# DIAGNijmegen/bodyct-dram-emph-subtype

Measured on AMD Instinct MI355X. Metric: CT volumes/sec (train step, 1x128x256x256), higher is better.
Workload: dtype f32; 1 GPU; BASELINE configs[1]: resnet18segcls train step (fwd+loss+bwd+Adam), batch 2/GPU, 1x128x256x256, fp32, inputs resident in HBM; global_batch=2, parallelism=dp1, hip_graph=False, streams=2

## Files before the change

bodyct-dram-emph-subtype_amd/csrc/conv_wino.hip:

```cpp
#include <stdio.h>
#include <stdlib.h>
#include <string.h>
#include "common.h"

namespace {

struct WinoGeom {
  int B, D, H, W;
  int d;
  int nz, ny, nx;
  int npts;
  int Tz, Ty, Tx;
  int T;
  int Tpad;
};

__device__ __forceinline__ void tile_origin(const WinoGeom& g, int t, int& b, int& z0, int& y0, int& x0) {
  int r = t;
  const int tx = r % g.Tx; r /= g.Tx;
  const int ty = r % g.Ty; r /= g.Ty;
  const int tz = r % g.Tz; r /= g.Tz;
  const int rx = r % g.d; r /= g.d;
  const int ry = r % g.d; r /= g.d;
  const int rz = r % g.d;
// ... 1432 lines not shown
  const int tid = threadIdx.x;
  const int lane = tid & 63;
  const int wave = __builtin_amdgcn_readfirstlane(tid >> 6);
  int L = xcd_remap(blockIdx.x, nblk);
  const int nt = L % n_tiles; L /= n_tiles;
  const int mt = L % m_tiles; L /= m_tiles;
  const int split = L % nsplit;
  const int xi = L / nsplit;
  const int t0 = split * kper;
  const int t1 = (t0 + kper < Tpad) ? t0 + kper : Tpad;
  int bcol = nt * BN + (lane % BQ) * 4;
  if (bcol > N - 4) bcol = N - 4;
  const float* Ab = Ah + (long)(lane / AQ) * M + mt * BM + (lane % AQ) * 4;
  const float* Bb = Bh + (long)(lane / BQ) * N + bcol;

  auto issue = [&](int it, int stage) __attribute__((always_inline)) {
    float* as = lds + stage * STAGE;
    float* bs = as + 32 * BM;
    const int tt = t0 + it * 32;
    const long row = ((long)(tt >> 8) * npts + xi) * 256 + (tt & 255);
    const float* ag = Ab + row * M;
    const float* bg = Bb + row * N;
#pragma unroll
    for (int j = 0; j < APW; ++j) {
      const int p = APW * wave + j;
      __builtin_amdgcn_global_load_lds((const __attribute__((address_space(1))) void*)(ag + (long)(p * ARPP) * M),
                                       (__attribute__((address_space(3))) void*)(as + p * 256), 16, 0, 0);
    }
#pragma unroll
    for (int jj = 0; jj < BPW; ++jj) {
      const int p = BPW * wave + jj;
      __builtin_amdgcn_global_load_lds((const __attribute__((address_space(1))) void*)(bg + (long)(p * BRPP) * N),
                                       (__attribute__((address_space(3))) void*)(bs + p * 256), 16, 0, 0);
    }
  };

  f32x16 acc[MI][NJ];
#pragma unroll
  for (int mi = 0; mi < MI; ++mi)
#pragma unroll
    for (int nj = 0; nj < NJ; ++nj)
#pragma unroll
      for (int e = 0; e < 16; ++e) acc[mi][nj][e] = 0.f;

  const int li = lane & 31, lh = lane >> 5;
  const int wm = wave % WMW, wn = wave / WMW;
  const int niter = (t1 - t0) / 32;

  if (niter > 0) issue(0, 0);
  for (int it = 0; it < niter; ++it) {
    __syncthreads();
    if (it + 1 < niter) issue(it + 1, (it + 1) & 1);
    const float* as = lds + (it & 1) * STAGE + wm * 32 * MI + li;
    const float* bs = lds + (it & 1) * STAGE + 32 * BM + wn * 32 * NJ + li;
#pragma unroll 4
    for (int kk = 0; kk < 16; ++kk) {
      const int kr = 2 * kk + lh;
      float af[MI], bf[NJ];
#pragma unroll
      for (int mi = 0; mi < MI; ++mi) af[mi] = as[kr * BM + mi * 32];
#pragma unroll
      for (int nj = 0; nj < NJ; ++nj) bf[nj] = bs[kr * BN + nj * 32];
#pragma unroll
      for (int nj = 0; nj < NJ; ++nj)
#pragma unroll
        for (int mi = 0; mi < MI; ++mi)
          acc[mi][nj] = __builtin_amdgcn_mfma_f32_32x32x2f32(af[mi], bf[nj], acc[mi][nj], 0, 0, 0);
    }
  }

  float* sb = slab + (((long)split * npts + xi) * M + mt * BM) * N + nt * BN;
#pragma unroll
  for (int mi = 0; mi < MI; ++mi)
#pragma unroll
    for (int e = 0; e < 16; ++e) {
      const int row = wm * 32 * MI + mi * 32 + (e & 3) + 8 * (e >> 2) + 4 * lh;
      float* o = sb + (long)row * N + wn * 32 * NJ + li;
#pragma unroll
      for (int nj = 0; nj < NJ; ++nj)
        if (nt * BN + wn * 32 * NJ + nj * 32 + li < N) o[nj * 32] = acc[mi][nj][e];
    }
}

__global__ __launch_bounds__(512, 2) void wino_gemm_tn64_kernel(const float* __restrict__ Ah, const float* __restrict__ Bh,
                                                                float* __restrict__ slab, const int Tpad, const int nsplit,
                                                                const int kper, const int nblk, const int npts) {
  constexpr int M = 64, N = 64, KS = 64;
  constexpr int STAGE = KS * (M + N);
  __shared__ __attribute__((aligned(1024))) float lds[2 * STAGE];
  const int tid = threadIdx.x, lane = tid & 63;
  const int wave = __builtin_amdgcn_readfirstlane(tid >> 6);
  int L = xcd_remap(blockIdx.x, nblk);
  const int split = L % nsplit;
  const int xi = L / nsplit;
  const int t0 = split * kper;
  const int t1 = (t0 + kper < Tpad) ? t0 + kper : Tpad;
  const int prow = lane >> 4, pcol = (lane & 15) * 4;
  auto issue = [&](int it, int stage) __attribute__((always_inline)) {
    float* as = lds + stage * STAGE;
    float* bs = as + KS * M;
    const int tt = t0 + it * KS;
    const long row = ((long)(tt >> 8) * npts + xi) * 256 + (tt & 255);
#pragma unroll
    for (int j = 0; j < 2; ++j) {
      const int p = 2 * wave + j;
      __builtin_amdgcn_global_load_lds((const __attribute__((address_space(1))) void*)(Ah + (row + p * 4 + prow) * M + pcol),
                                       (__attribute__((address_space(3))) void*)(as + p * 256), 16, 0, 0);
      __builtin_amdgcn_global_load_lds((const __attribute__((address_space(1))) void*)(Bh + (row + p * 4 + prow) * N + pcol),
                                       (__attribute__((address_space(3))) void*)(bs + p * 256), 16, 0, 0);
    }
  };
  f32x16 acc;
#pragma unroll
  for (int e = 0; e < 16; ++e) acc[e] = 0.f;
  const int li = lane & 31, lh = lane >> 5;
  const int wm = wave & 1, wn = (wave >> 1) & 1, kh = wave >> 2;
  const int niter = (t1 - t0) / KS;
  if (niter > 0) issue(0, 0);
  for (int it = 0; it < niter; ++it) {
    __syncthreads();
    if (it + 1 < niter) issue(it + 1, (it + 1) & 1);
    const float* as = lds + (it & 1) * STAGE + (kh * 32) * M + wm * 32 + li;
    const float* bs = lds + (it & 1) * STAGE + KS * M + (kh * 32) * N + wn * 32 + li;
#pragma unroll 4
    for (int kk = 0; kk < 16; ++kk) {
      const int kr = 2 * kk + lh;
      acc = __builtin_amdgcn_mfma_f32_32x32x2f32(as[kr * M], bs[kr * N], acc, 0, 0, 0);
    }
  }
  __syncthreads();
  float* ex = lds + (wave & 3) * 1024;
  if (kh == 1) {
#pragma unroll
    for (int e = 0; e < 16; ++e) ex[e * 64 + lane] = acc[e];
  }
  __syncthreads();
  if (kh == 0) {
    float* sb = slab + (((long)split * npts + xi) * M) * N;
#pragma unroll
    for (int e = 0; e < 16; ++e) {
      const int row = wm * 32 + (e & 3) + 8 * (e >> 2) + 4 * lh;
      sb[(long)row * N + wn * 32 + li] = acc[e] + ex[e * 64 + lane];
    }
  }
}

typedef short s16x4 __attribute__((ext_vector_type(4)));
typedef short s16x8 __attribute__((ext_vector_type(8)));

template <int WMW, int MI, int NJ, int NT>
__global__ __launch_bounds__(512) void wino_gemm_tn_bf16_kernel(const float* __restrict__ Ah, const float* __restrict__ Bh,
                                                                float* __restrict__ slab, const int Tpad, const int M,
                                                                const int N, const int m_tiles, const int n_tiles,
                                                                const int nsplit, const int kper, const int nblk,
                                                                const int npts) {
  constexpr int WNW = 8 / WMW;
  constexpr int BM = WMW * 32 * MI, BN = WNW * 32 * NJ;
  static_assert(BM % 64 == 0 && BM <= 256 && BN % 64 == 0 && BN <= 256, "one DMA piece = 256 floats");
  constexpr int STAGE = 32 * (BM + BN);
  constexpr int AQ = BM / 4, ARPP = 64 / AQ, APW = BM / 64;
  constexpr int BQ = BN / 4, BRPP = 64 / BQ, BPW = BN / 64;
  __shared__ __attribute__((aligned(1024))) float lds[2 * STAGE];

  const int tid = threadIdx.x;
  const int lane = tid & 63;
  const int wave = __builtin_amdgcn_readfirstlane(tid >> 6);
// ... 118 lines not shown
      for (int nj = 0; nj < NJ; ++nj)
        if (nt * BN + wn * 32 * NJ + nj * 32 + li < N) o[nj * 32] = acc[mi][nj][e];
    }
}

#define WINO_TILING_DISPATCH(g_, CALL_)                                 \
  do {                                                                  \
    if ((g_).nz == 4 && (g_).ny == 4 && (g_).nx == 4) { CALL_(4, 4, 4); } \
    else if ((g_).nz == 4 && (g_).ny == 4) { CALL_(4, 4, 2); }          \
    else if ((g_).nz == 4) { CALL_(4, 2, 2); }                          \
    else { CALL_(2, 2, 2); }                                            \
  } while (0)
int math_mode() {
  const char* e = tune_env("DRAM_MATH");
  if (!e) return 0;
  if (!strcmp(e, "bf16x3")) return 1;
  if (!strcmp(e, "bf16")) return 2;
  return 0;
}

bool wino_geom_ok(const DramConvDesc* d) {
  if (!d) return false;
  if (d->B < 1 || d->D < 1 || d->H < 1 || d->W < 1) return false;
  if (d->k != 3 || d->stride != 1 || d->dil < 1 || d->pad != d->dil) return false;
  if (d->Do != d->D || d->Ho != d->H || d->Wo != d->W) return false;
  if (d->Cin < 64 || d->Cout < 64 || d->Cin % 64 != 0 || d->Cout % 64 != 0) return false;
  return true;
}

long long tiles_for(const DramConvDesc* d, int nz, int ny, int nx) {
  const int dd = d->dil;
  auto tiles = [&](int n, int per) { return (long long)(((n + dd - 1) / dd + per - 1) / per); };
  return (long long)d->B * dd * dd * dd * tiles(d->D, nz) * tiles(d->H, ny) * tiles(d->W, nx);
}

void pick_tiling(const DramConvDesc* d, const int pass, int& nz, int& ny, int& nx) {
  static const int cand[4][3] = {{4, 4, 4}, {4, 4, 2}, {4, 2, 2}, {2, 2, 2}};
  if (const char* e = tune_env("DRAM_WINO_TILING")) {
    int a = 0, b = 0, c = 0;
    if (sscanf(e, "%d,%d,%d", &a, &b, &c) == 3)
      for (int i = 0; i < 4; ++i)
        if (cand[i][0] == a && cand[i][1] == b && cand[i][2] == c) { nz = a; ny = b; nx = c; return; }
  }
  if (math_mode() == 2) { nz = ny = nx = 2; return; }
  (void)pass;
  long long best = -1;
  int bi = 3;
  for (int i = 0; i < 4; ++i) {
    const long long T = tiles_for(d, cand[i][0], cand[i][1], cand[i][2]);
    const long long Tpad = (T + 255) / 256 * 256;
    if (i < 3 && Tpad < 512) continue;
    const long long cost = (long long)(cand[i][0] + 2) * (cand[i][1] + 2) * (cand[i][2] + 2) * (Tpad + T);
    if (best < 0 || cost < best) { best = cost; bi = i; }
  }
  nz = cand[bi][0]; ny = cand[bi][1]; nx = cand[bi][2];
}

WinoGeom make_geom(const DramConvDesc* d, const int pass = 0) {
  WinoGeom g{};
  g.B = d->B; g.D = d->D; g.H = d->H; g.W = d->W; g.d = d->dil;
  pick_tiling(d, pass, g.nz, g.ny, g.nx);
  g.npts = (g.nz + 2) * (g.ny + 2) * (g.nx + 2);
  auto tiles = [&](int n, int per) { return ((n + g.d - 1) / g.d + per - 1) / per; };
  g.Tz = tiles(g.D, g.nz); g.Ty = tiles(g.H, g.ny); g.Tx = tiles(g.W, g.nx);
  const long long T = (long long)g.B * g.d * g.d * g.d * g.Tz * g.Ty * g.Tx;
  g.T = (int)T;
  g.Tpad = (int)((T + 255) / 256 * 256);
  return g;
}

bool wino_size_ok(const DramConvDesc* d) {
  const long long cmax = d->Cin > d->Cout ? d->Cin : d->Cout;
  for (int pass = 0; pass < 2; ++pass) {
    const WinoGeom g = make_geom(d, pass);
    const long long T = (long long)g.B * g.d * g.d * g.d * g.Tz * g.Ty * g.Tx;
    if (!(T > 0 && (T + 255) * cmax < (1LL << 31))) return false;
  }
  const long long plane_b = (long long)d->H * d->W * cmax * 4;
  if ((5LL * d->dil + 1) * plane_b >= (1LL << 30) || 216LL * 256 * cmax * 4 >= (1LL << 30)) return false;
  return true;
}


struct TnPlan { int bm, bn, m_tiles, n_tiles, nsplit, kper; };
bool plan_tn(const DramConvDesc* d, const WinoGeom& g, TnPlan& p) {
  const int M = d->Cout, N = d->Cin;
  p.bm = M % 256 == 0 ? 256 : (M % 128 == 0 ? 128 : 64);
  const int ncand = p.bm == 256 ? 3 : 2;
  const int cand[3] = {256, 128, 64};
  p.bn = 0;
  int best_pad = 1 << 30;
  for (int i = 0; i < ncand; ++i) {
    const int padded = (N + cand[i] - 1) / cand[i] * cand[i];
    if (padded * 100 <= N * 113) { p.bn = cand[i]; break; }
    if (padded < best_pad) { best_pad = padded; p.bn = cand[i]; }
  }
  p.m_tiles = M / p.bm;
  p.n_tiles = (N + p.bn - 1) / p.bn;
  if (p.bn >= 128 && (p.bn > 128 || p.bm == 256)) {
    const long w1 = (long)g.npts * p.m_tiles * p.n_tiles;
    const int hb = p.bn / 2, hn = (N + hb - 1) / hb;
    const long w2 = (long)g.npts * p.m_tiles * hn;
    if (w1 >= 512 && (double)((w2 + 255) / 256) * 0.5 * 1.03 < (double)((w1 + 255) / 256)) {
      p.bn = hb;
      p.n_tiles = hn;
    }
  }
  const int base = g.npts * p.m_tiles * p.n_tiles;
  const int k32 = g.Tpad / 32;
  int ns = 1;
  while (base * ns < (g.npts == 1 ? 256 : 512) && ns * 2 <= k32 / 4 && ns < (g.npts == 1 ? 256 : 16)) ns *= 2;
  p.nsplit = ns;
  p.kper = ((k32 + ns - 1) / ns) * 32;
  return true;
}

int wino_nt() {
  static const int v = tune_env("DRAM_WINO_NT") ? atoi(tune_env("DRAM_WINO_NT")) : 3;
  return v;
}

int grid_for(long waves) {
  long b = (waves + 3) / 4;
  return (int)(b > 65536 ? 65536 : (b < 1 ? 1 : b));
}

template <int MODE>
int launch_wino_in(const float* src, float* dst, const WinoGeom& g, const int C, const int math, hipStream_t s,
                   const float* pscale = nullptr, const float* pshift = nullptr, const int Cd = 0, const int cofs = 0) {
  const long units = (long)g.Tpad * (C / 64);
  if (Cd && (math || !(g.nz == 4 && g.ny == 4 && g.nx == 4) || C % 64 || cofs % 64 || cofs + C > Cd)) return DRAM_ERR_UNSUPPORTED;
  if (pscale) {
    if (MODE != 0 || math || !pshift || !(g.nz == 4 && g.ny == 4 && g.nx == 4)) return DRAM_ERR_UNSUPPORTED;
    const double in_elems = (double)g.B * g.D * g.H * g.W * C;
    DramProf prof(DRAM_FAM_WINO_IN, 9444, 0.0, 4.0 * (in_elems + (double)g.npts * g.Tpad * C), s);
    if constexpr (MODE == 0) {
      if (wino_nt() & 1) hipLaunchKernelGGL((wino_in444_kernel<0, false, true, true>), dim3(grid_for(2 * units)), dim3(256), 0, s, src, dst, g, C, pscale, pshift, Cd, cofs);
      else hipLaunchKernelGGL((wino_in444_kernel<0, false, false, true>), dim3(grid_for(2 * units)), dim3(256), 0, s, src, dst, g, C, pscale, pshift, Cd, cofs);
    }
    DRAM_LAUNCH_CHECK();
    return DRAM_OK;
  }
  const double in_elems = (double)g.B * g.D * g.H * g.W * C;
  DramProf prof(DRAM_FAM_WINO_IN, MODE * 1000 + g.nz * 100 + g.ny * 10 + g.nx, 0.0,
                4.0 * (in_elems + (double)g.npts * g.Tpad * C), s);
  static const int half = tune_env("DRAM_WINO_HALF") ? atoi(tune_env("DRAM_WINO_HALF")) : 1;
  if ((half || Cd) && g.nz == 4 && g.ny == 4 && g.nx == 4) {
    if (math) hipLaunchKernelGGL((wino_in444_kernel<MODE, true, false>), dim3(grid_for(2 * units)), dim3(256), 0, s, src, dst, g, C, nullptr, nullptr, 0, 0);
    else if (wino_nt() & 1) hipLaunchKernelGGL((wino_in444_kernel<MODE, false, true>), dim3(grid_for(2 * units)), dim3(256), 0, s, src, dst, g, C, nullptr, nullptr, Cd, cofs);
    else hipLaunchKernelGGL((wino_in444_kernel<MODE, false, false>), dim3(grid_for(2 * units)), dim3(256), 0, s, src, dst, g, C, nullptr, nullptr, Cd, cofs);
    DRAM_LAUNCH_CHECK();
    return DRAM_OK;
  }
#define W_IN1(NZ_, NY_, NX_)                                                                                       \
  do {                                                                                                             \
    if (math)                                                                                                      \
      hipLaunchKernelGGL((wino_in_kernel<MODE, NZ_, NY_, NX_, true>), dim3(grid_for(units)), dim3(256), 0, s, src, dst, g, C);  \
    else                                                                                                           \
      hipLaunchKernelGGL((wino_in_kernel<MODE, NZ_, NY_, NX_, false>), dim3(grid_for(units)), dim3(256), 0, s, src, dst, g, C); \
  } while (0)
  WINO_TILING_DISPATCH(g, W_IN1);
#undef W_IN1
  DRAM_LAUNCH_CHECK();
  return DRAM_OK;
}

int run_nn(const float* A, const float* U, float* Y, const WinoGeom& g, int N, int K, hipStream_t s,
           const GemmEpilogue ep = GemmEpilogue{nullptr, nullptr, nullptr, nullptr}, const int math = 0,
           const bool alone = true) {
  const int m_tiles = g.Tpad / 256;
  int nj = 1;
  double best = 1e30;
  for (int c = 4; c >= 1; c >>= 1) {
    if (N % (64 * c) != 0) continue;
    const long wgs = (long)g.npts * m_tiles * (N / (64 * c));
    const double cost = (double)((wgs + 255) / 256) * c * (c == 4 ? 1.0 : (c == 2 ? 1.03 : 1.10));
    if (cost < best) { best = cost; nj = c; }
  }
  if (const char* e = tune_env("DRAM_NN_NJ")) { const int v = atoi(e); if ((v == 1 || v == 2 || v == 4) && N % (64 * v) == 0) nj = v; }
  const int n_tiles = N / (64 * nj);
  const int nblk = g.npts * m_tiles * n_tiles;
  DramProf prof(DRAM_FAM_WINO_GEMM_NN, nj, 2.0 * g.npts * (double)g.Tpad * N * K,
                4.0 * g.npts * ((double)g.Tpad * (K + N) + (double)N * K), s,
                g.npts > 1 ? 2.0 * g.B * g.D * g.H * g.W * (double)N * K * 27.0 : -1.0);
  if (math) {
#define WNB(NJ_, NT_)                                                                                                  \
  hipLaunchKernelGGL((wino_gemm_nn_bf16_kernel<NJ_, NT_>), dim3(nblk), dim3(512), 0, s, A, U, Y, g.Tpad, N, K, m_tiles, \
                     n_tiles, nblk, g.npts)
    if (math == 1) { if (nj == 4) WNB(4, 3); else if (nj == 2) WNB(2, 3); else WNB(1, 3); }
    else { if (nj == 4) WNB(4, 1); else if (nj == 2) WNB(2, 1); else WNB(1, 1); }
#undef WNB
    DRAM_LAUNCH_CHECK();
    return DRAM_OK;
  }
#define WNN(NJ_)                                                                                                   \
  hipLaunchKernelGGL((wino_gemm_nn_kernel<NJ_>), dim3(nblk), dim3(512), 0, s, A, U, Y, g.Tpad, N, K, m_tiles, n_tiles, \
                     nblk, g.npts, ep, epi_lds)
// ... 127 lines not shown
  if (d->Cin < 64 || d->Cout < 64 || d->Cin % 64 != 0 || d->Cout % 64 != 0) return false;
  const long long M = (long long)d->B * d->D * d->H * d->W;
  const long long cmax = d->Cin > d->Cout ? d->Cin : d->Cout;
  return M % 256 == 0 && M * cmax < (1LL << 31);
}
WinoGeom c1_geom(const DramConvDesc* d) {
  WinoGeom g{};
  g.B = d->B; g.D = d->D; g.H = d->H; g.W = d->W; g.d = 1;
  g.nz = g.ny = g.nx = 1;
  g.npts = 1;
  g.T = g.Tpad = d->B * d->D * d->H * d->W;
  return g;
}
__global__ __launch_bounds__(256) void slab_sum_kernel(const float* __restrict__ slab, float* __restrict__ out, const long n,
                                                       const int nsplit) {
  __shared__ float part[4][64];
  const int r = threadIdx.x & 63, kg = threadIdx.x >> 6;
  for (long i0 = blockIdx.x * 64L; i0 < n; i0 += (long)gridDim.x * 64L) {
    const long i = i0 + r;
    const bool live = i < n;
    float p[8];
#pragma unroll
    for (int j = 0; j < 8; ++j) p[j] = 0.f;
    if (live) {
      int k = kg;
      for (; k + 28 < nsplit; k += 32) {
#pragma unroll
        for (int j = 0; j < 8; ++j) p[j] += slab[(long)(k + 4 * j) * n + i];
      }
      for (int j = 0; k < nsplit; k += 4, ++j) p[j] += slab[(long)k * n + i];
    }
    part[kg][r] = ((p[0] + p[1]) + (p[2] + p[3])) + ((p[4] + p[5]) + (p[6] + p[7]));
    __syncthreads();
    if (kg == 0 && live) out[i] = (part[0][r] + part[1][r]) + (part[2][r] + part[3][r]);
    __syncthreads();
  }
}
}

extern "C" int dram_conv1x1_applicable(const DramConvDesc* d) { return c1_ok(d) ? 1 : 0; }

extern "C" int dram_conv1x1_num_stat_rows(const DramConvDesc* d) {
  if (!c1_ok(d)) return DRAM_ERR_UNSUPPORTED;
  return c1_geom(d).Tpad / 256;
}

extern "C" int dram_conv1x1_fwd(const float* x, const float* w2d, const float* bias, float* y, float* stats_partial,
                                const DramConvDesc* d, dram_stream_t stream) {
  if (!x || !w2d || !y) return DRAM_ERR_BAD_ARG;
  if (!c1_ok(d)) return DRAM_ERR_UNSUPPORTED;
  return run_nn(x, w2d, y, c1_geom(d), d->Cout, d->Cin, (hipStream_t)stream,
                GemmEpilogue{bias, nullptr, nullptr, stats_partial});
}

extern "C" int dram_conv1x1_bwd_data(const float* dy, const float* wt, float* dx, const float* add, const float* gate,
                                     const DramConvDesc* d, dram_stream_t stream) {
  if (!dy || !wt || !dx || (gate && !add)) return DRAM_ERR_BAD_ARG;
  if (!c1_ok(d)) return DRAM_ERR_UNSUPPORTED;
  return run_nn(dy, wt, dx, c1_geom(d), d->Cin, d->Cout, (hipStream_t)stream, GemmEpilogue{nullptr, add, gate, nullptr});
}

extern "C" size_t dram_conv1x1_bwd_weight_workspace(const DramConvDesc* d) {
  if (!c1_ok(d)) return 0;
  TnPlan p;
  plan_tn(d, c1_geom(d), p);
  return (size_t)p.nsplit * d->Cout * d->Cin * sizeof(float);
}

extern "C" int dram_conv1x1_bwd_weight(const float* x, const float* dy, float* dw, const DramConvDesc* d, void* workspace,
                                       size_t workspace_bytes, dram_stream_t stream) {
  if (!x || !dy || !dw) return DRAM_ERR_BAD_ARG;
  if (!c1_ok(d)) return DRAM_ERR_UNSUPPORTED;
  const WinoGeom g = c1_geom(d);
  TnPlan p;
  plan_tn(d, g, p);
  const size_t need = (size_t)p.nsplit * d->Cout * d->Cin * sizeof(float);
  if (p.nsplit > 1 && (!workspace || workspace_bytes < need)) return DRAM_ERR_WORKSPACE;
  hipStream_t s = (hipStream_t)stream;
  float* slab = p.nsplit > 1 ? (float*)workspace : dw;
  const int nblk = p.nsplit * p.m_tiles * p.n_tiles;
  {
  DramProf prof(DRAM_FAM_WINO_GEMM_TN, p.bm * 1000 + p.bn, 2.0 * (double)g.Tpad * d->Cout * d->Cin,
                4.0 * ((double)g.Tpad * (d->Cout + d->Cin) + (double)p.nsplit * d->Cout * d->Cin), s);
#define C1TN(WM_, MI_, NJ_)                                                                                         \
  hipLaunchKernelGGL((wino_gemm_tn_kernel<WM_, MI_, NJ_>), dim3(nblk), dim3(512), 0, s, dy, x, slab, g.Tpad, d->Cout, \
                     d->Cin, p.m_tiles, p.n_tiles, p.nsplit, p.kper, nblk, 1)
  if (p.bm == 256 && p.bn == 256) C1TN(4, 2, 4);
  else if (p.bm == 256 && p.bn == 128) C1TN(4, 2, 2);
  else if (p.bm == 256 && p.bn == 64) C1TN(4, 2, 1);
  else if (p.bm == 128 && p.bn == 256) C1TN(2, 2, 2);
  else if (p.bm == 128 && p.bn == 128) C1TN(2, 2, 1);
  else if (p.bm == 64 && p.bn == 256) C1TN(2, 1, 2);
  else if (p.bm == 64 && p.bn == 128) C1TN(2, 1, 1);
  else return DRAM_ERR_UNSUPPORTED;
#undef C1TN
  DRAM_LAUNCH_CHECK();
  }
  if (p.nsplit > 1) {
    const long n = (long)d->Cout * d->Cin;
    const int grid = (int)((n + 63) / 64 > 4096 ? 4096 : (n + 63) / 64);
    DramProf prof(DRAM_FAM_WINO_WGRAD_OUT, 0, 0.0, 4.0 * (double)n * (p.nsplit + 1), s);
    hipLaunchKernelGGL(slab_sum_kernel, dim3(grid), dim3(256), 0, s, slab, dw, n, p.nsplit);
    DRAM_LAUNCH_CHECK();
  }
  return DRAM_OK;
}

extern "C" int dram_wino_applicable(const DramConvDesc* d) {
  return (wino_geom_ok(d) && wino_size_ok(d)) ? 1 : 0;
}

static double fill(double wgs, double slots) {
  if (wgs < 1.0) wgs = 1.0;
  const double rounds = (double)(long)((wgs + slots - 1.0) / slots);
  return wgs / (rounds * slots);
}
static double wino_cost_per_voxel(double K, double N, double tpad, double npts, double pv) {
  const double nt = (double)(long)((N + 255.0) / 256.0);
  const double gemm = 2.0 * pv * K * N / (118e12 * fill(npts * (tpad / 256.0) * nt, 256.0));
  const double traffic = 4.0 * pv * (K + N) / 4.7e12;
  const double in_rate = npts > 200.0 ? 4.0e12 : 4.9e12;
  return (4.0 + 4.0 * pv) * K / in_rate + (gemm > traffic ? gemm : traffic) + (4.0 + 4.0 * pv) * N / 3.4e12;
}
static double direct_rate(const DramConvDesc* d, double N) {
  const double lat = d->dil;
  const double sz = (double)(long)((d->D + lat - 1) / lat), sy = (double)(long)((d->H + lat - 1) / lat),
               sx = (double)(long)((d->W + lat - 1) / lat);
  const double mt = d->B * lat * lat * lat * (double)(long)((sz + 3) / 4) * (double)(long)((sy + 7) / 8) *
                    (double)(long)((sx + 7) / 8);
  return 135e12 * fill(mt * (double)(long)((N + 127.0) / 128.0), 512.0);
}

extern "C" int dram_conv_algo(const DramConvDesc* d) {
  const char* v = tune_env("DRAM_CONV_ALGO");
  const int algo = v ? atoi(v) : 0;
  if (algo == 1) return 0;
  if (c1_ok(d)) return 3;
  const bool w3 = dram_wino_applicable(d) != 0, w2 = dram_wino2d_applicable(d) != 0;
  if (algo == 2) return w3 ? 1 : 0;
  if (algo == 3) return w2 ? 2 : 0;
  const double vox = d ? (double)d->B * d->D * d->H * d->W : 0.0;
  double best = 1e30;
  int pick = 0;
  if (w3) {
    const WinoGeom g = make_geom(d, 0), gb = make_geom(d, 1);
    if (g.T >= 128) {
      const double vpad = (double)g.nz * g.ny * g.nx * g.Tpad, pv = g.npts / ((double)g.nz * g.ny * g.nx);
      const double vpadb = (double)gb.nz * gb.ny * gb.nx * gb.Tpad, pvb = gb.npts / ((double)gb.nz * gb.ny * gb.nx);
      const double direct = vox * 54.0 * d->Cin * d->Cout * 0.5 *
                            (1.0 / direct_rate(d, d->Cout) + 1.0 / direct_rate(d, d->Cin));
      const double wino = 0.5 * (vpad * wino_cost_per_voxel(d->Cin, d->Cout, g.Tpad, g.npts, pv) +
                                 vpadb * wino_cost_per_voxel(d->Cout, d->Cin, gb.Tpad, gb.npts, pvb));
      if (wino < 0.92 * direct) { best = wino; pick = 1; }
    }
  }
  if (w2 && d->D >= 12 && vox >= 65536.0) {
    const int zt = (d->D + 15) / 16 * 16;
    const double rf = d->Cout % 64 == 0 ? 200e12 : 155e12, rb = d->Cin % 64 == 0 ? 200e12 : 155e12;
    const double w2d = vox * zt / d->D * 54.0 * d->Cin * d->Cout * 0.5 * (1.0 / rf + 1.0 / rb);
    const double direct = vox * 54.0 * d->Cin * d->Cout / 135e12;
    const char* me = tune_env(d->D >= 64 ? "DRAM_W2D_MARGIN_BIG" : "DRAM_W2D_MARGIN");
    const bool tolerant = (d->flags & DRAM_CONV_ROUNDING_TOLERANT) != 0;
    const double margin = me ? atof(me) : ((d->D >= 64 || tolerant) ? 1.0 : 1.15);
    if (w2d < 0.92 * direct && w2d < margin * best) { best = w2d; pick = 2; }
  }
  return pick;
}

constexpr double W2D_WGRAD_RATE = 240e12;
// ... 101 lines not shown
  if (!dram_wino_applicable(d) || math_mode()) return 0;
  const WinoGeom g = make_geom(d, 0);
  return (g.nz == 4 && g.ny == 4 && g.nx == 4) ? 1 : 0;
}

extern "C" int dram_wino_conv3d_fwd_bn(const float* x_pre, const float* pscale, const float* pshift, const float* uf,
                                       const float* bias, float* y, float* stats_partial, float* v_keep,
                                       const DramConvDesc* d, void* workspace, size_t workspace_bytes, dram_stream_t stream) {
  if (!x_pre || !pscale || !pshift || !uf || !y) return DRAM_ERR_BAD_ARG;
  if (!dram_wino_prologue_supported(d)) return DRAM_ERR_UNSUPPORTED;
  return run_conv(x_pre, uf, bias, nullptr, nullptr, y, stats_partial, v_keep, d, 0, d->Cin, d->Cout, workspace,
                  workspace_bytes, (hipStream_t)stream, pscale, pshift);
}

extern "C" int dram_wino_conv3d_fwd_cat(const float* x0, int C0, const float* x1, int C1, const float* uf, const float* bias,
                                        float* y, float* stats_partial, float* v_keep, const DramConvDesc* d,
                                        void* workspace, size_t workspace_bytes, dram_stream_t stream) {
  if (!x0 || !x1 || !uf || !y || !d || C0 < 64 || C1 < 64 || (C0 % 64) || (C1 % 64) || C0 + C1 != d->Cin)
    return DRAM_ERR_BAD_ARG;
  if (!dram_wino_prologue_supported(d)) return DRAM_ERR_UNSUPPORTED;
  return run_conv(x0, uf, bias, nullptr, nullptr, y, stats_partial, v_keep, d, 0, d->Cin, d->Cout, workspace,
                  workspace_bytes, (hipStream_t)stream, nullptr, nullptr, x1, C0);
}

extern "C" size_t dram_wino_v_elems(const DramConvDesc* d) {
  if (!dram_wino_applicable(d)) return 0;
  const WinoGeom g = make_geom(d);
  return (size_t)g.npts * g.Tpad * (size_t)d->Cin;
}

extern "C" int dram_wino_conv3d_bwd_data(const float* dy, const float* ub, float* dx, const float* add,
                                         const float* gate, const DramConvDesc* d, void* workspace,
                                         size_t workspace_bytes, dram_stream_t stream) {
  if (!dy || !ub || !dx || (gate && !add)) return DRAM_ERR_BAD_ARG;
  if (!dram_wino_applicable(d)) return DRAM_ERR_UNSUPPORTED;
  return run_conv(dy, ub, nullptr, add, gate, dx, nullptr, nullptr, d, 1, d->Cout, d->Cin, workspace, workspace_bytes,
                  (hipStream_t)stream);
}

extern "C" int dram_wino_num_stat_rows_bwd(const DramConvDesc* d) {
  if (!dram_wino_applicable(d)) return 0;
  const WinoGeom g = make_geom(d, 1);
  return (g.T + wino_tpb(g.T) - 1) / wino_tpb(g.T);
}

extern "C" int dram_wino_conv3d_bwd_data_bn(const float* dy, const float* ub, float* dx, const float* bn_y,
                                            const float* bn_mean, const float* bn_invstd, const float* bn_scale,
                                            const float* bn_shift, float* stats_partial, const DramConvDesc* d,
                                            void* workspace, size_t workspace_bytes, dram_stream_t stream) {
  if (!dy || !ub || !dx || !bn_y || !bn_mean || !bn_invstd || !bn_scale || !bn_shift || !stats_partial)
    return DRAM_ERR_BAD_ARG;
  if (!dram_wino_applicable(d) || d->Cin % 64) return DRAM_ERR_UNSUPPORTED;
  return run_conv(dy, ub, nullptr, nullptr, nullptr, dx, stats_partial, nullptr, d, 1, d->Cout, d->Cin, workspace,
                  workspace_bytes, (hipStream_t)stream, nullptr, nullptr, nullptr, 0,
                  BnBwdStat{bn_y, bn_mean, bn_invstd, bn_scale, bn_shift});
}

extern "C" int dram_wino_conv3d_bwd_weight(const float* x, const float* v_cache, const float* dy, float* dw,
                                           const DramConvDesc* d, void* workspace, size_t workspace_bytes,
                                           dram_stream_t stream) {
  if ((!x && !v_cache) || !dy || !dw) return DRAM_ERR_BAD_ARG;
  if (!dram_wino_applicable(d)) return DRAM_ERR_UNSUPPORTED;
  const WinoGeom g = make_geom(d);
  TnPlan p;
  if (!plan_tn(d, g, p)) return DRAM_ERR_UNSUPPORTED;
  const size_t need = dram_wino_workspace(d, 2);
  if (!workspace || workspace_bytes < need) return DRAM_ERR_WORKSPACE;
  hipStream_t s = (hipStream_t)stream;
  float* V = (float*)workspace;
  float* Dh = V + (size_t)g.npts * g.Tpad * d->Cin;
  float* slab = Dh + (size_t)g.npts * g.Tpad * d->Cout;
  const int math = math_mode();
  if (v_cache) V = const_cast<float*>(v_cache);
  else {
    const int rc0 = launch_wino_in<0>(x, V, g, d->Cin, math, s);
    if (rc0 != DRAM_OK) return rc0;
  }
  { const int rc1 = launch_wino_in<1>(dy, Dh, g, d->Cout, math, s); if (rc1 != DRAM_OK) return rc1; }
  const int nblk = g.npts * p.nsplit * p.m_tiles * p.n_tiles;
  {
  DramProf prof(DRAM_FAM_WINO_GEMM_TN, p.bm * 1000 + p.bn, 2.0 * g.npts * (double)g.Tpad * d->Cout * d->Cin,
                4.0 * g.npts * ((double)g.Tpad * (d->Cout + d->Cin) + (double)p.nsplit * d->Cout * d->Cin), s,
                2.0 * g.B * g.D * g.H * g.W * (double)d->Cout * d->Cin * 27.0);
#define WTN(WM_, MI_, NJ_)                                                                                             \
  do {                                                                                                                 \
    if (math == 1)                                                                                                     \
      hipLaunchKernelGGL((wino_gemm_tn_bf16_kernel<WM_, MI_, NJ_, 3>), dim3(nblk), dim3(512), 0, s, Dh, V, slab, g.Tpad, \
                         d->Cout, d->Cin, p.m_tiles, p.n_tiles, p.nsplit, p.kper, nblk, g.npts);                       \
    else if (math == 2)                                                                                                \
      hipLaunchKernelGGL((wino_gemm_tn_bf16_kernel<WM_, MI_, NJ_, 1>), dim3(nblk), dim3(512), 0, s, Dh, V, slab, g.Tpad, \
                         d->Cout, d->Cin, p.m_tiles, p.n_tiles, p.nsplit, p.kper, nblk, g.npts);                       \
    else                                                                                                               \
      hipLaunchKernelGGL((wino_gemm_tn_kernel<WM_, MI_, NJ_>), dim3(nblk), dim3(512), 0, s, Dh, V, slab, g.Tpad,       \
                         d->Cout, d->Cin, p.m_tiles, p.n_tiles, p.nsplit, p.kper, nblk, g.npts);                       \
  } while (0)
  static const int tn64 = tune_env("DRAM_TN64") ? atoi(tune_env("DRAM_TN64")) : 1;
  if (tn64 && math == 0 && d->Cout == 64 && d->Cin == 64 && p.kper % 64 == 0 && g.Tpad % 64 == 0)
    hipLaunchKernelGGL(wino_gemm_tn64_kernel, dim3(g.npts * p.nsplit), dim3(512), 0, s, Dh, V, slab, g.Tpad, p.nsplit,
                       p.kper, g.npts * p.nsplit, g.npts);
  else if (p.bm == 256 && p.bn == 256) WTN(4, 2, 4);
  else if (p.bm == 256 && p.bn == 128) WTN(4, 2, 2);
  else if (p.bm == 256 && p.bn == 64) WTN(4, 2, 1);
  else if (p.bm == 128 && p.bn == 256) WTN(2, 2, 2);
  else if (p.bm == 128 && p.bn == 128) WTN(2, 2, 1);
  else if (p.bm == 64 && p.bn == 256) WTN(2, 1, 2);
  else if (p.bm == 64 && p.bn == 128) WTN(2, 1, 1);
  else return DRAM_ERR_UNSUPPORTED;
#undef WTN
  DRAM_LAUNCH_CHECK();
  }
  const long n = (long)d->Cout * d->Cin;
  DramProf prof(DRAM_FAM_WINO_WGRAD_OUT, 1, 0.0, 4.0 * (double)n * ((double)g.npts * p.nsplit + 27.0), s);
#define W_WGO(NZ_, NY_, NX_)                                                                                         \
  hipLaunchKernelGGL((wino_wgrad_out_kernel<NZ_, NY_, NX_>), dim3((unsigned)((n + 63) / 64)), dim3(512), 0, s, slab, dw, \
                     d->Cout, d->Cin, p.nsplit)
  WINO_TILING_DISPATCH(g, W_WGO);
#undef W_WGO
  DRAM_LAUNCH_CHECK();
  return DRAM_OK;
}
```

bodyct-dram-emph-subtype_amd/ops.py:

```python
from __future__ import annotations

import contextlib
import ctypes
import os
import threading
import weakref
from dataclasses import dataclass
from typing import Dict, List, Optional, Tuple

import torch

from . import _lib
from ._lib import DramConvDesc

Tensor = torch.Tensor


def _L():
    return _lib.load()


_TLS = threading.local()


# ... 231 lines not shown
        return self.out(self.H)

    @property
    def Wo(self):
        return self.out(self.W)

    @property
    def taps(self):
        return self.k ** 3

    @property
    def flops(self) -> float:
        return 2.0 * self.B * self.Do * self.Ho * self.Wo * self.Cout * self.Cin * self.taps

    @property
    def in_shape(self):
        return (self.B, self.D, self.H, self.W, self.Cin)

    @property
    def out_shape(self):
        return (self.B, self.Do, self.Ho, self.Wo, self.Cout)

    def desc(self) -> DramConvDesc:
        return DramConvDesc(self.B, self.D, self.H, self.W, self.Cin, self.Do, self.Ho, self.Wo, self.Cout,
                            self.k, self.stride, self.pad, self.dil, self.tol)


_CAPTURE_KEEP: List[object] = []
_CAPTURE_OWNER: Optional[List[object]] = None


@contextlib.contextmanager
def capture_keepalive(owner: List[object]):
    global _CAPTURE_OWNER
    prev, _CAPTURE_OWNER = _CAPTURE_OWNER, owner
    try:
        yield owner
    finally:
        _CAPTURE_OWNER = prev


def capture_id() -> int:
    return int(_L().dram_stream_capture_id(_stream()))


def _keep_for_capture(obj):
    keep = _CAPTURE_OWNER if _CAPTURE_OWNER is not None else _CAPTURE_KEEP
    if not any(o is obj for o in keep[-16:]):
        keep.append(obj)


_WORKSPACE: Dict[tuple, Tensor] = {}
_CAPTURE_WS: Dict[tuple, "weakref.ref"] = {}


def _workspace(nbytes: int, device) -> Tensor:
    device = torch.device(device)
    n = (nbytes + 3) // 4
    cid = capture_id()
    if cid:
        key = (device, _stream().value, cid)
        ref = _CAPTURE_WS.get(key)
        ws = ref() if ref is not None else None
        if ws is None or ws.numel() < n:
            ws = torch.empty((n,), device=device, dtype=torch.float32)
            _keep_for_capture(ws)
            for k in [k for k, r in _CAPTURE_WS.items() if r() is None]:
                del _CAPTURE_WS[k]
            _CAPTURE_WS[key] = weakref.ref(ws)
        return ws
    key = (device, _stream().value)
    ws = _WORKSPACE.pop(key, None)
    if ws is None or ws.numel() < n:
        ws = None
        ws = torch.empty((n,), device=device, dtype=torch.float32)
        while len(_WORKSPACE) >= 6:
            _WORKSPACE.pop(next(iter(_WORKSPACE)))
    _WORKSPACE[key] = ws
    return ws


_PLAN_ENV = ("DRAM_CONV_ALGO", "DRAM_WINO_TILING", "DRAM_MATH", "DRAM_W2D_V", "DRAM_IGEMM_V", "DRAM_IGEMM_V3_FORCE",
             "DRAM_WGRAD_V", "DRAM_BF16_NW", "DRAM_BF16_WGRAD", "DRAM_W2D_MARGIN", "DRAM_W2D_MARGIN_BIG", "DRAM_NN_STREAM",
             "DRAM_WGRAD_MARGIN")


class ConvPlan:
    __slots__ = ("desc", "dref", "desc_ovl", "dref_ovl", "algo", "walgo", "taps_f", "taps_b", "stat_rows", "ws_fwd", "ws_bwd", "ws_wgrad",
                 "v_elems", "ws_direct_wgrad", "bf16", "bf16_stat_rows", "bf16_ws_wgrad", "prologue")

    def __init__(self, g: "ConvGeom"):
        L = _L()
        self.desc = g.desc()
        self.dref = d = ctypes.byref(self.desc)
        self.desc_ovl = g.desc()
        self.desc_ovl.flags |= _lib.DRAM_CONV_BWD_OVERLAPPED
        self.dref_ovl = ctypes.byref(self.desc_ovl)
        self.algo = int(L.dram_conv_algo(d))
        self.walgo = int(L.dram_conv_wgrad_algo(d))
        if self.algo == 1:
            self.taps_f, self.taps_b = int(L.dram_wino_num_points(d)), int(L.dram_wino_num_points_bwd(d))
        else:
            self.taps_f = self.taps_b = 48 if self.algo == 2 else g.taps
        self.stat_rows = int({0: L.dram_conv_num_mtiles, 1: L.dram_wino_num_stat_rows, 2: L.dram_wino2d_num_stat_rows,
                              3: L.dram_conv1x1_num_stat_rows}[self.algo](d))
        self.ws_fwd = int(L.dram_wino_workspace(d, 0)) if self.algo == 1 else 0
        self.ws_bwd = int(L.dram_wino_workspace(d, 1)) if self.algo == 1 else 0
        self.v_elems = int(L.dram_wino_v_elems(d)) if (self.algo == 1 or self.walgo == 1) else 0
        self.ws_wgrad = {3: lambda: int(L.dram_conv1x1_bwd_weight_workspace(d)),
                         2: lambda: int(L.dram_wgrad_w2d_workspace(d)),
                         1: lambda: int(L.dram_wino_workspace(d, 2))}.get(self.walgo, lambda: 0)()
        self.ws_direct_wgrad = int(L.dram_conv3d_bwd_weight_workspace(d)) if (self.walgo == 0 or self.ws_wgrad == 0) else 0
        self.prologue = bool(self.algo == 1 and L.dram_wino_prologue_supported(d))
        self.bf16 = bool(L.dram_conv_bf16_supported(d))
        self.bf16_stat_rows = int(L.dram_conv_bf16_num_stat_rows(d)) if self.bf16 else 0
        self.bf16_ws_wgrad = int(L.dram_conv3d_bwd_weight_bf16_workspace(d)) if self.bf16 else 0


_PLANS: Dict[tuple, ConvPlan] = {}


def conv_plan(g: "ConvGeom") -> ConvPlan:
    env = os.environ
    key = (g,) + tuple(env.get(k) for k in _PLAN_ENV) if env.get("DRAM_TUNING") == "1" else g
    p = _PLANS.get(key)
    if p is None:
        p = _PLANS[key] = ConvPlan(g)
    return p


def conv_algo(g: "ConvGeom") -> int:
    return conv_plan(g).algo


def conv_use_wino(g: "ConvGeom") -> bool:
    return conv_algo(g) == 1


def packed_taps(g: "ConvGeom", bwd: bool = False) -> int:
    p = conv_plan(g)
    return p.taps_b if bwd else p.taps_f


def s2_geom(g: "ConvGeom") -> Optional["ConvGeom"]:
    if (g.k != 3 or g.stride != 2 or g.pad != 1 or g.dil != 1 or ((g.D | g.H | g.W) & 1) or g.Cin % 8
            or tuning_env("DRAM_BF16_S2", "1") == "0"):
        return None
    g8 = ConvGeom(g.B, g.D // 2, g.H // 2, g.W // 2, 8 * g.Cin, g.Cout, 3, 1, 1, 1, g.tol)
    return g8 if (conv_plan(g8).bf16 and tuple(g8.out_shape) == tuple(g.out_shape)) else None


def s2d(x: Tensor) -> Tensor:
    B, D, H, W, C = x.shape
    x8 = torch.empty((B, D // 2, H // 2, W // 2, 8 * C), device=x.device, dtype=BF16)
    _chk(_L().dram_s2d_bf16(_p(x), _p(x8), B, D, H, W, C, _stream()), "dram_s2d_bf16")
    return x8


def pack_conv_weight(w: Tensor, want_fwd=True, want_bwd=True, g: Optional["ConvGeom"] = None, dtype=torch.float32
                     ) -> Tuple[Optional[Tensor], Optional[Tensor]]:
    _req(w, "w")
    Cout, Cin = w.shape[0], w.shape[1]
    taps = w.shape[2] * w.shape[3] * w.shape[4]
    if dtype == BF16 and g is not None and conv_plan(g).bf16:
        wf = torch.empty((taps, Cout, Cin), device=w.device, dtype=BF16) if want_fwd else None
        wb = torch.empty((taps, Cin, Cout), device=w.device, dtype=BF16) if want_bwd else None
        _chk(_L().dram_pack_conv_weight_bf16(_p(w), _p(wf), _p(wb), Cout, Cin, taps, _stream()), "dram_pack_conv_weight_bf16")
# ... 851 lines not shown
```

Before: 55.73 volumes/sec.

## Add persistent multi-stage TN GEMM kernel for Winograd weight-gradient

Adds a persistent-block variant of the TN (weight-gradient) Winograd GEMM. Each block loops over several tile/split work items, keeping a 2-3 stage LDS ring of async global-to-LDS loads so the next item's loads overlap the current item's MFMA work and store. The grid is sized to the number of resident block slots. It is on by default for the fp32 Winograd weight-gradient path, and an optional mode rebalances the split-K count. The aim is to cut tail and launch-wave inefficiency and prologue/epilogue stalls, at the cost of more complex control flow and possible LDS or occupancy pressure.

Result: no change. 55.65 volumes/sec (-0.2%).

```diff
diff --git a/bodyct-dram-emph-subtype_amd/csrc/conv_wino.hip b/bodyct-dram-emph-subtype_amd/csrc/conv_wino.hip
--- a/bodyct-dram-emph-subtype_amd/csrc/conv_wino.hip
+++ b/bodyct-dram-emph-subtype_amd/csrc/conv_wino.hip
@@ -1538,6 +1538,182 @@
     }
 }
 
+template <int WMW, int MI, int NJ>
+__global__ __launch_bounds__(512, (3 * 32 * (WMW * 32 * MI + (8 / WMW) * 32 * NJ) * 4 <= 80 * 1024) ? 2 : 1)
+void wino_gemm_tn_pers_kernel(const float* __restrict__ Ah, const float* __restrict__ Bh, float* __restrict__ slab,
+                              const int Tpad, const int M, const int N, const int m_tiles, const int n_tiles,
+                              const int nsplit, const int kper, const int nblk, const int npts) {
+  constexpr int WNW = 8 / WMW;
+  constexpr int BM = WMW * 32 * MI, BN = WNW * 32 * NJ;
+  static_assert(BM % 64 == 0 && BM <= 256 && BN % 64 == 0 && BN <= 256, "one DMA piece = 256 floats");
+  constexpr int STAGE = 32 * (BM + BN);
+  constexpr int AQ = BM / 4, ARPP = 64 / AQ, APW = BM / 64;
+  constexpr int BQ = BN / 4, BRPP = 64 / BQ, BPW = BN / 64;
+  constexpr int S = (3 * STAGE * 4 <= 160 * 1024) ? 3 : 2;
+  constexpr int AHEAD = (APW + BPW) * (S - 2);
+  __shared__ __attribute__((aligned(1024))) float ring[S * STAGE];
+
+  const int tid = threadIdx.x;
+  const int lane = tid & 63;
+  const int wave = __builtin_amdgcn_readfirstlane(tid >> 6);
+  const int li = lane & 31, lh = lane >> 5;
+  const int wm = wave % WMW, wn = wave / WMW;
+  const int G = gridDim.x;
+
+  struct Item { int idx, xi, split, mt, nt, t0, niter; };
+  auto item_of = [&](int idx) __attribute__((always_inline)) {
+    Item q;
+    q.idx = idx;
+    int L = xcd_remap(idx, nblk);
+    q.nt = L % n_tiles; L /= n_tiles;
+    q.mt = L % m_tiles; L /= m_tiles;
+    q.split = L % nsplit;
+    q.xi = L / nsplit;
+    q.t0 = q.split * kper;
+    const int t1 = (q.t0 + kper < Tpad) ? q.t0 + kper : Tpad;
+    q.niter = t1 > q.t0 ? (t1 - q.t0) / 32 : 0;
+    return q;
+  };
+  auto item_from = [&](int idx) __attribute__((always_inline)) {
+    Item q;
+    q.idx = idx;
+    q.niter = 0;
+    while (idx < nblk) {
+      q = item_of(idx);
+      if (q.niter > 0) break;
+      idx += G;
+      q.idx = idx;
+    }
+    return q;
+  };
+  auto store = [&](const Item& q, const f32x16 (&acc)[MI][NJ]) __attribute__((always_inline)) {
+    float* sb = slab + (((long)q.split * npts + q.xi) * M + q.mt * BM) * N + q.nt * BN;
+#pragma unroll
+    for (int mi = 0; mi < MI; ++mi)
+#pragma unroll
+      for (int e = 0; e < 16; ++e) {
+        const int row = wm * 32 * MI + mi * 32 + (e & 3) + 8 * (e >> 2) + 4 * lh;
+        float* o = sb + (long)row * N + wn * 32 * NJ + li;
+#pragma unroll
+        for (int nj = 0; nj < NJ; ++nj)
+          if (q.nt * BN + wn * 32 * NJ + nj * 32 + li < N) o[nj * 32] = acc[mi][nj][e];
+      }
+  };
+
+  f32x16 acc[MI][NJ];
+#pragma unroll
+  for (int mi = 0; mi < MI; ++mi)
+#pragma unroll
+    for (int nj = 0; nj < NJ; ++nj)
+#pragma unroll
+      for (int e = 0; e < 16; ++e) acc[mi][nj][e] = 0.f;
+
+  if ((long)nsplit * kper > Tpad) {
+    for (int idx = blockIdx.x; idx < nblk; idx += G) {
+      const Item q = item_of(idx);
+      if (q.niter == 0) store(q, acc);
+    }
+  }
+
+  Item ic = item_from(blockIdx.x);
+  if (ic.idx >= nblk) return;
+  Item cc = ic;
+  int i_it = 0, c_it = 0;
+
+  auto stage_of = [&](int k) __attribute__((always_inline)) -> float* { return ring + k * STAGE; };
+  bool i_more = true;
+  auto issue_next = [&](float* stage) __attribute__((always_inline)) {
+    float* as = stage;
+    float* bs = stage + 32 * BM;
+    const int tt = ic.t0 + i_it * 32;
+    const long row = ((long)(tt >> 8) * npts + ic.xi) * 256 + (tt & 255);
+    int bcol = ic.nt * BN + (lane % BQ) * 4;
+    if (bcol > N - 4) bcol = N - 4;
+    const float* ag = Ah + (row + lane / AQ) * M + ic.mt * BM + (lane % AQ) * 4;
+    const float* bg = Bh + (row + lane / BQ) * N + bcol;
+#pragma unroll
+    for (int j = 0; j < APW; ++j) {
+      const int p = APW * wave + j;
+      __builtin_amdgcn_global_load_lds((const __attribute__((address_space(1))) void*)(ag + (long)(p * ARPP) * M),
+                                       (__attribute__((address_space(3))) void*)(as + p * 256), 16, 0, 0);
+    }
+#pragma unroll
+    for (int jj = 0; jj < BPW; ++jj) {
+      const int p = BPW * wave + jj;
+      __builtin_amdgcn_global_load_lds((const __attribute__((address_space(1))) void*)(bg + (long)(p * BRPP) * N),
+                                       (__attribute__((address_space(3))) void*)(bs + p * 256), 16, 0, 0);
+    }
+    if (i_more && i_it + 1 == ic.niter) {
+      const Item nx = item_from(ic.idx + G);
+      if (nx.idx < nblk) {
+        ic = nx;
+        i_it = 0;
+      } else {
+        i_more = false;
+      }
+    } else if (i_more) {
+      ++i_it;
+    }
+  };
+  auto wait_next = [&]() __attribute__((always_inline)) {
+    __builtin_amdgcn_s_waitcnt(0x0F70 | (AHEAD & 15) | ((AHEAD >> 4) << 14));
+    asm volatile("" ::: "memory");
+  };
+  auto compute = [&](const float* st) __attribute__((always_inline)) {
+    const float* as = st + lh * BM + wm * 32 * MI + li;
+    const float* bs = st + 32 * BM + lh * BN + wn * 32 * NJ + li;
+    float af[2][MI], bf[2][NJ];
+    auto frag = [&](int kk, int buf) __attribute__((always_inline)) {
+#pragma unroll
+      for (int mi = 0; mi < MI; ++mi) af[buf][mi] = as[2 * kk * BM + mi * 32];
+#pragma unroll
+      for (int nj = 0; nj < NJ; ++nj) bf[buf][nj] = bs[2 * kk * BN + nj * 32];
+    };
+    frag(0, 0);
+#pragma unroll
+    for (int kk = 0; kk < 16; ++kk) {
+      if (kk + 1 < 16) frag(kk + 1, (kk + 1) & 1);
+#pragma unroll
+      for (int nj = 0; nj < NJ; ++nj)
+#pragma unroll
+        for (int mi = 0; mi < MI; ++mi)
+          acc[mi][nj] = __builtin_amdgcn_mfma_f32_32x32x2f32(af[kk & 1][mi], bf[kk & 1][nj], acc[mi][nj], 0, 0, 0);
+      if (kk + 1 < 16) __builtin_amdgcn_sched_group_barrier(0x100, MI + NJ, 0);
+      __builtin_amdgcn_sched_group_barrier(0x008, MI * NJ, 0);
+      __builtin_amdgcn_sched_barrier(0);
+    }
+  };
+
+  issue_next(stage_of(0));
+  if (S == 3) issue_next(stage_of(1));
+  wait_next();
+  for (;;) {
+#pragma unroll
+    for (int k = 0; k < S; ++k) {
+      asm volatile("" ::: "memory");
+      __builtin_amdgcn_s_barrier();
+      issue_next(stage_of((k + S - 1) % S));
+      compute(stage_of(k));
+      wait_next();
+      if (++c_it == cc.niter) {
+        store(cc, acc);
+#pragma unroll
+        for (int mi = 0; mi < MI; ++mi)
+#pragma unroll
+          for (int nj = 0; nj < NJ; ++nj)
+#pragma unroll
+            for (int e = 0; e < 16; ++e) acc[mi][nj][e] = 0.f;
+        cc = item_from(cc.idx + G);
+        c_it = 0;
+        if (cc.idx >= nblk) {
+          __builtin_amdgcn_s_waitcnt(0x0F70);
+          return;
+        }
+      }
+    }
+  }
+}
+
 __global__ __launch_bounds__(512, 2) void wino_gemm_tn64_kernel(const float* __restrict__ Ah, const float* __restrict__ Bh,
                                                                 float* __restrict__ slab, const int Tpad, const int nsplit,
                                                                 const int kper, const int nblk, const int npts) {
@@ -1822,6 +1998,12 @@
 }
 
 
+int tn_persist() {
+  const char* e = tune_env("DRAM_TN_PERSIST");
+  return e ? atoi(e) : 1;
+}
+bool tn_use_pers(int bm, int bn) { return tn_persist() != 0 && !(bm == 64 && bn == 256); }
+
 struct TnPlan { int bm, bn, m_tiles, n_tiles, nsplit, kper; };
 bool plan_tn(const DramConvDesc* d, const WinoGeom& g, TnPlan& p) {
   const int M = d->Cout, N = d->Cin;
@@ -1850,9 +2032,31 @@
   const int k32 = g.Tpad / 32;
   int ns = 1;
   while (base * ns < (g.npts == 1 ? 256 : 512) && ns * 2 <= k32 / 4 && ns < (g.npts == 1 ? 256 : 16)) ns *= 2;
+  if (tn_persist() >= 2 && math_mode() == 0 && g.npts > 1 && p.bm >= 128 && tn_use_pers(p.bm, p.bn)) {
+    long best_cost = -1;
+    int best = ns;
+    for (int c = 1; c <= ns; c *= 2) {
+      const long cost = (long)(((long)base * c + 255) / 256) * ((k32 + c - 1) / c + 3);
+      if (best_cost < 0 || cost < best_cost) { best_cost = cost; best = c; }
+    }
+    ns = best;
+  }
   p.nsplit = ns;
   p.kper = ((k32 + ns - 1) / ns) * 32;
   return true;
+}
+
+int tn_pers_grid(int nblk, int bm, int bn) {
+  const int slots = 256 * ((3 * 32 * (bm + bn) * 4 <= 80 * 1024) ? 2 : 1);
+  const int rounds = (nblk + slots - 1) / slots;
+  int grid = ((nblk + rounds - 1) / rounds + 7) / 8 * 8;
+  if (grid > slots) grid = slots;
+  if (grid > nblk) grid = nblk;
+  if (const char* e = tune_env("DRAM_TN_GRID")) {
+    const int v = atoi(e);
+    if (v >= 1 && v < grid) grid = v;
+  }
+  return grid;
 }
 
 int wino_nt() {
@@ -2146,9 +2350,18 @@
   {
   DramProf prof(DRAM_FAM_WINO_GEMM_TN, p.bm * 1000 + p.bn, 2.0 * (double)g.Tpad * d->Cout * d->Cin,
                 4.0 * ((double)g.Tpad * (d->Cout + d->Cin) + (double)p.nsplit * d->Cout * d->Cin), s);
-#define C1TN(WM_, MI_, NJ_)                                                                                         \
-  hipLaunchKernelGGL((wino_gemm_tn_kernel<WM_, MI_, NJ_>), dim3(nblk), dim3(512), 0, s, dy, x, slab, g.Tpad, d->Cout, \
-                     d->Cin, p.m_tiles, p.n_tiles, p.nsplit, p.kper, nblk, 1)
+  const char* c1e = tune_env("DRAM_TN_C1");
+  const bool persist = tn_use_pers(p.bm, p.bn) && c1e && atoi(c1e) == 1;
+  const int pgrid = tn_pers_grid(nblk, p.bm, p.bn);
+#define C1TN(WM_, MI_, NJ_)                                                                                           \
+  do {                                                                                                                \
+    if (persist)                                                                                                      \
+      hipLaunchKernelGGL((wino_gemm_tn_pers_kernel<WM_, MI_, NJ_>), dim3(pgrid), dim3(512), 0, s, dy, x, slab, g.Tpad, \
+                         d->Cout, d->Cin, p.m_tiles, p.n_tiles, p.nsplit, p.kper, nblk, 1);                           \
+    else                                                                                                              \
+      hipLaunchKernelGGL((wino_gemm_tn_kernel<WM_, MI_, NJ_>), dim3(nblk), dim3(512), 0, s, dy, x, slab, g.Tpad,      \
+                         d->Cout, d->Cin, p.m_tiles, p.n_tiles, p.nsplit, p.kper, nblk, 1);                           \
+  } while (0)
   if (p.bm == 256 && p.bn == 256) C1TN(4, 2, 4);
   else if (p.bm == 256 && p.bn == 128) C1TN(4, 2, 2);
   else if (p.bm == 256 && p.bn == 64) C1TN(4, 2, 1);
@@ -2416,13 +2629,18 @@
   DramProf prof(DRAM_FAM_WINO_GEMM_TN, p.bm * 1000 + p.bn, 2.0 * g.npts * (double)g.Tpad * d->Cout * d->Cin,
                 4.0 * g.npts * ((double)g.Tpad * (d->Cout + d->Cin) + (double)p.nsplit * d->Cout * d->Cin), s,
                 2.0 * g.B * g.D * g.H * g.W * (double)d->Cout * d->Cin * 27.0);
+  const bool persist = tn_use_pers(p.bm, p.bn);
+  const int pgrid = tn_pers_grid(nblk, p.bm, p.bn);
 #define WTN(WM_, MI_, NJ_)                                                                                             \
   do {                                                                                                                 \
-    if (math == 1)                                                                                                     \
+    if (math == 1)                                                                                                  \
       hipLaunchKernelGGL((wino_gemm_tn_bf16_kernel<WM_, MI_, NJ_, 3>), dim3(nblk), dim3(512), 0, s, Dh, V, slab, g.Tpad, \
                          d->Cout, d->Cin, p.m_tiles, p.n_tiles, p.nsplit, p.kper, nblk, g.npts);                       \
     else if (math == 2)                                                                                                \
       hipLaunchKernelGGL((wino_gemm_tn_bf16_kernel<WM_, MI_, NJ_, 1>), dim3(nblk), dim3(512), 0, s, Dh, V, slab, g.Tpad, \
+                         d->Cout, d->Cin, p.m_tiles, p.n_tiles, p.nsplit, p.kper, nblk, g.npts);                       \
+    else if (persist)                                                                                                  \
+      hipLaunchKernelGGL((wino_gemm_tn_pers_kernel<WM_, MI_, NJ_>), dim3(pgrid), dim3(512), 0, s, Dh, V, slab, g.Tpad, \
                          d->Cout, d->Cin, p.m_tiles, p.n_tiles, p.nsplit, p.kper, nblk, g.npts);                       \
     else                                                                                                               \
       hipLaunchKernelGGL((wino_gemm_tn_kernel<WM_, MI_, NJ_>), dim3(nblk), dim3(512), 0, s, Dh, V, slab, g.Tpad,       \
diff --git a/bodyct-dram-emph-subtype_amd/ops.py b/bodyct-dram-emph-subtype_amd/ops.py
--- a/bodyct-dram-emph-subtype_amd/ops.py
+++ b/bodyct-dram-emph-subtype_amd/ops.py
@@ -337,7 +337,7 @@
 
 _PLAN_ENV = ("DRAM_CONV_ALGO", "DRAM_WINO_TILING", "DRAM_MATH", "DRAM_W2D_V", "DRAM_IGEMM_V", "DRAM_IGEMM_V3_FORCE",
              "DRAM_WGRAD_V", "DRAM_BF16_NW", "DRAM_BF16_WGRAD", "DRAM_W2D_MARGIN", "DRAM_W2D_MARGIN_BIG", "DRAM_NN_STREAM",
-             "DRAM_WGRAD_MARGIN")
+             "DRAM_WGRAD_MARGIN", "DRAM_TN_PERSIST")
 
 
 class ConvPlan:
```
